# ppjian19/PhoreGen

Measured on AMD Instinct MI355X. Metric: denoise-steps/sec (batch=128, ~40-atom graphs), higher is better.
Workload: dtype f32; 1 GPU; BASELINE.json configs[2]: ONE batch of 128 LigPhore-shaped graphs (n~N(40,6) atoms, p~N(107,30) pharmacophore nodes), partitioned over 1 GPU(s) by the fitted step cost, steps t=999.. of the 1000-step sampler, device Philox noise, trajectory written; graphs_total=128, graphs_rank0=128, n_ctx=18401, n_lig=5115, e_knn=588832, e_bond=203720, e3=8087028, parallelism=graph-sharded x1, final RCCL gather only, triplet_workgroups_rank0=256

## Files before the change

### include/phoregen_hip.h

```cpp
#ifndef PHOREGEN_HIP_H
#define PHOREGEN_HIP_H

#include <stdint.h>

#ifdef __cplusplus
extern "C" {
#endif

const char* pg_last_error(void);
int pg_abi_version(void);
int pg_abi_struct_sizes(int* out, int n);

int pg_order_point_create(void** ev);
int pg_order_point_destroy(void* ev);
int pg_order_point_record(void* ev, void* stream);
int pg_order_point_wait(void* ev, void* stream);
int pg_debug_order_point_fence_free(int on);

enum {
  PG_OP_RECORD = 0, PG_OP_WAIT = 1, PG_OP_GEMM = 2, PG_OP_SEG_ATTN = 3, PG_OP_EMBED_CTX = 4, PG_OP_EMBED_BOND = 5, PG_OP_KNN_CTX = 6,
  PG_OP_LIG_NORMALS = 7, PG_OP_EDGE_GATE = 8, PG_OP_KNN_GROUP_BY_KIND = 9, PG_OP_BOND_SMEAR = 10, PG_OP_ATTN_FOLD_QUERY = 11,
  PG_OP_ATTN_UNFOLD_VALUE = 12, PG_OP_APPLY_DX = 13, PG_OP_LAYER_GEOM = 14, PG_OP_ROWS_LINEAR = 15, PG_OP_ATOM_COUNT = 16,
  PG_OP_EMBED_BOND_E16 = 17
};
// ... 12 lines not shown
int pg_program_destroy(void* prog);

int pg_micro_mfma_f32(int workgroups, int iters, float* sink, double* flops, void* stream);

int pg_selftest_mfma(int* d_result, void* stream);
int pg_selftest_philox(const uint32_t* ctr_key, int n, uint32_t* out, void* stream);
int pg_debug_force_generic_seg(int mask);

typedef struct {
  const float* X;   int ldx;  int K1;
  const float* X2;  int ldx2; int K2;
  const float* W;   int ldw;
  const float* bias;
  const float* ln_gamma; const float* ln_beta;
  const float* add1; int ld_add1; const int* idx1;
  const float* add2; int ld_add2; const int* idx2;
  float out_scale;
  int   act;
  float* Y; int ldy; int M; int N;
  const int* rows;
  int add_rows;
  int row_extent;
  const int* tile_rows;
} PgGemm;
int pg_gemm(const PgGemm* p, void* stream);
int pg_debug_gemm_streaming(int on);
int pg_gemm_is_streaming(const PgGemm* p);

typedef struct {
  int n_graphs, n_ctx, n_lig, n_phore, n_bond;
  int max_nlig;
  int max_gctx;
  const int* g_ctx_off;
  const int* g_nph;
  const int* g_nlig;
  const int* g_eid_off;
  const int* eid;
  const int* ctx_graph;
  const uint8_t* ctx_is_lig;
  const int* lig2ctx;
  const int* bond_src;
  const int* bond_dst;
  const int* bond_desc;
  const int* g_bond_off;
  const int* edge_ref;
} PgTopo;
// ... 492 lines not shown
```

### phoregen_amd/csrc/gemm.hip

```cpp
#include <stdlib.h>

#include "common.h"
#include "../../include/phoregen_hip.h"

namespace pg {

constexpr int BM = 128, BN = 128, BK = 32, LDT = BK + 1;


__global__ __launch_bounds__(256) void gemm_kernel(PgGemm p PG_ABL_PARAM) {
  __shared__ __attribute__((aligned(16))) float smem[(BM + BN) * LDT];
  float* const As = smem;
  float* const Bs = smem + BM * LDT;
  __shared__ float rstat[BM * 2];

  const int tid = threadIdx.x, lane = tid & 63, wave = tid >> 6;
  const int col0 = blockIdx.x * BN;
  const int K = p.K1 + p.K2;
  for (int rb = blockIdx.y; rb * BM < p.M; rb += gridDim.y) {
  const int row0 = rb * BM;
  const int wr = (wave >> 1) * 64, wc = (wave & 1) * 64;
  const bool ln = p.ln_gamma != nullptr;

  if (ln) {
// ... 197 lines not shown
      const int src = rows ? rows[grow] : grow;
      *reinterpret_cast<f4*>(xs + r * RL_LD + 4 * c4) = __builtin_nontemporal_load(reinterpret_cast<const f4*>(X + (size_t)src * ldx) + c4);
    }
    __syncthreads();
    f4 acc = {bias, bias, bias, bias};
    const float* xa = xs + (16 * wave + m) * RL_LD + g;
#pragma unroll
    for (int s_ = 0; s_ < 32; ++s_) acc = mfma16(xa[4 * s_], wr[s_], acc);
    if (m < n_out) {
#pragma unroll
      for (int r = 0; r < 4; ++r) {
        const int grow = row0 + 16 * wave + 4 * g + r;
        if (grow < M) Y[(size_t)grow * ldy + m] = acc[r];
      }
    }
  }
}

}

namespace pg {
bool gemm_stream_eligible(const PgGemm* p);
bool gemm_stream_windows_ok(const PgGemm* p);
int launch_gemm_stream(const PgGemm* p, hipStream_t st);
}

static int g_gemm_stream = 1;
extern "C" int pg_debug_gemm_streaming(int on) { const int old = g_gemm_stream; g_gemm_stream = on; return old; }

extern "C" int pg_gemm_is_streaming(const PgGemm* p) {
  return p && (p->tile_rows || (g_gemm_stream && pg::gemm_stream_eligible(p))) ? 1 : 0;
}

extern "C" int pg_gemm(const PgGemm* p, void* stream) {
  if (!p || !p->X || !p->W || !p->Y || p->M < 0 || p->N <= 0) { pg::set_error("pg_gemm: bad arguments"); return PG_ERR_ARG; }
  if (p->M == 0) return PG_OK;
  if (p->K2 > 0 && !p->X2) { pg::set_error("pg_gemm: K2 > 0 without X2"); return PG_ERR_ARG; }
  if (p->ln_gamma && !p->ln_beta) { pg::set_error("pg_gemm: ln_gamma without ln_beta"); return PG_ERR_ARG; }
  if (p->ln_gamma && (p->K2 != 0 || p->K1 != 128 || (p->ldx & 3) || ((size_t)p->X & 15))) { pg::set_error("pg_gemm: LayerNorm-on-load needs K1 == 128, K2 == 0, 16-byte aligned rows"); return PG_ERR_ARG; }
  if (p->tile_rows) {
    if (!pg::gemm_stream_windows_ok(p)) {
      pg::set_error("pg_gemm: tile_rows needs the streaming kernel's plain or LayerNorm-on-load form (K1 = 128, K2 = 0, no added operand, "
                    "no rows, act = 0, N a multiple of 128), M = 64 x windows and row_extent >= 64 (M %d, N %d, K1 %d, K2 %d, row_extent %d)",
                    p->M, p->N, p->K1, p->K2, p->row_extent);
      return PG_ERR_ARG;
    }
    hipPointerAttribute_t at;
    if (hipPointerGetAttributes(&at, p->tile_rows) != hipSuccess || at.type == hipMemoryTypeUnregistered) {
      (void)hipGetLastError();
      pg::set_error("pg_gemm: tile_rows is not device-accessible memory");
      return PG_ERR_ARG;
    }
    if (at.type == hipMemoryTypeHost || at.type == hipMemoryTypeManaged) {
      const int* o = p->tile_rows;
      for (int t = 0; t < p->M / 64; ++t)
        if (o[t] < 0 || o[t] > p->row_extent - 64) {
          pg::set_error("pg_gemm: tile_rows[%d] = %d outside [0, row_extent - 64 = %d]", t, o[t], p->row_extent - 64);
          return PG_ERR_ARG;
        }
    }
    return pg::launch_gemm_stream(p, (hipStream_t)stream);
  }
// ... 22 lines not shown
```

### phoregen_amd/csrc/gemm_stream.hip

```cpp
#include <type_traits>

#include "wave_prims.h"
#include "../../include/phoregen_hip.h"

namespace pg {

typedef int i2v __attribute__((ext_vector_type(2)));

constexpr int ST_BM = 64;
constexpr int ST_STAGE = ST_BM * 128 * 4;

template <int NW , int NADD , int K1 ,
          int K2 , bool LN ,
          bool SSP = false ,
          bool WIN = false >
__global__ __launch_bounds__(NW * 64, NW == 4 ? 2 : 1) void gemm_stream_kernel(PgGemm p, int n_tiles) {
  extern __shared__ __attribute__((aligned(1024))) char st_lds[];
  const int lane = threadIdx.x & 63;
  const int wave = __builtin_amdgcn_readfirstlane(threadIdx.x >> 6);
  const int l31 = lane & 31, kh = lane >> 5;
  const int colw = blockIdx.y * (NW * 32) + 32 * wave;
  const int col = colw + l31;

  constexpr bool DMA = K1 == 128;
  static_assert((K1 == 128 || K1 == 16 || K1 == 0) && (K2 == 20 || K2 == 0) && K1 + K2 > 0, "K1 128 | 16 | 0, K2 20 | 0");
  float Wr[DMA ? 64 : 1];
  if constexpr (DMA) {
    const float* wrow = p.W + (size_t)col * p.ldw + 4 * kh;
#pragma unroll
    for (int c = 0; c < 16; ++c) {
      const f4 w = *reinterpret_cast<const f4*>(wrow + 8 * c);
#pragma unroll
      for (int e = 0; e < 4; ++e) Wr[4 * c + e] = w[e];
    }
  }
  float W2r[K2 ? 10 : 1];
  if constexpr (K2 > 0) {
#pragma unroll
    for (int s2 = 0; s2 < 10; ++s2) W2r[s2] = p.W[(size_t)col * p.ldw + K1 + 10 * kh + s2];
  }
  const unsigned ldx2b = (unsigned)p.ldx2 * 4u;
  const __amdgpu_buffer_rsrc_t descX2 = __builtin_amdgcn_make_buffer_rsrc(const_cast<float*>(K2 ? p.X2 : nullptr), 0, (unsigned)p.M * ldx2b, 0x00020000);
  const unsigned voffX2 = (unsigned)l31 * ldx2b + 40u * kh;
  float xa[2][10], xb[2][10];
  auto load_x2 = [&](unsigned row0, float (&x)[2][10]) {
#pragma unroll
    for (int b = 0; b < 2; ++b) {
      const unsigned so = (row0 + 32u * b) * ldx2b;
      const i4v v0 = __builtin_amdgcn_raw_buffer_load_b128(descX2, voffX2, so, 0);
      const i4v v1 = __builtin_amdgcn_raw_buffer_load_b128(descX2, voffX2 + 16u, so, 0);
      const i2v v2 = __builtin_amdgcn_raw_buffer_load_b64(descX2, voffX2 + 32u, so, 0);
#pragma unroll
      for (int e = 0; e < 4; ++e) { x[b][e] = __builtin_bit_cast(float, (int)v0[e]); x[b][4 + e] = __builtin_bit_cast(float, (int)v1[e]); }
      x[b][8] = __builtin_bit_cast(float, (int)v2[0]);
      x[b][9] = __builtin_bit_cast(float, (int)v2[1]);
    }
// ... 1 lines not shown
  float W1r[K1 == 16 ? 8 : 1];
  float xra[2][8], xrb[2][8];
  const unsigned ldxrb = K1 == 16 ? (unsigned)p.ldx * 4u : 0u;
  const __amdgpu_buffer_rsrc_t descXr = __builtin_amdgcn_make_buffer_rsrc(const_cast<float*>(K1 == 16 ? p.X : nullptr), 0, (unsigned)p.M * ldxrb, 0x00020000);
  const unsigned voffXr = (unsigned)l31 * ldxrb + 32u * kh;
  if constexpr (K1 == 16) {
#pragma unroll
    for (int s1 = 0; s1 < 8; ++s1) W1r[s1] = p.W[(size_t)col * p.ldw + 8 * kh + s1];
  }
  auto load_xr = [&](unsigned row0, float (&x)[2][8]) {
#pragma unroll
    for (int b = 0; b < 2; ++b) {
      const unsigned so = (row0 + 32u * b) * ldxrb;
      const i4v v0 = __builtin_amdgcn_raw_buffer_load_b128(descXr, voffXr, so, 0);
      const i4v v1 = __builtin_amdgcn_raw_buffer_load_b128(descXr, voffXr + 16u, so, 0);
#pragma unroll
      for (int e = 0; e < 4; ++e) { x[b][e] = __builtin_bit_cast(float, (int)v0[e]); x[b][4 + e] = __builtin_bit_cast(float, (int)v1[e]); }
    }
  };
  const float bias = p.bias ? p.bias[col] : 0.f;
  f16v biasv;
#pragma unroll
  for (int r = 0; r < 16; ++r) biasv[r] = bias;

  const f4* const lnt = reinterpret_cast<const f4*>(st_lds + 2 * ST_STAGE);
  if constexpr (LN) {
    float* t = reinterpret_cast<float*>(st_lds + 2 * ST_STAGE);
    if (threadIdx.x < 128) { t[threadIdx.x] = p.ln_gamma[threadIdx.x]; t[128 + threadIdx.x] = p.ln_beta[threadIdx.x]; }
    __syncthreads();
  }

  const unsigned ldxb = (unsigned)p.ldx * 4u, ldyb = (unsigned)p.ldy * 4u;
  const unsigned n_rows = WIN ? (unsigned)p.row_extent : (unsigned)p.M;
  const i4v descX = raw_buffer_desc(p.X, n_rows * ldxb);
  const __amdgpu_buffer_rsrc_t descY = __builtin_amdgcn_make_buffer_rsrc(p.Y, 0, n_rows * ldyb, 0x00020000);
  const unsigned row_sub = lane >> 3, pp = lane & 7;
  const unsigned voff_even = row_sub * ldxb + ((pp ^ ((row_sub >> 1) & 7u)) << 4);
  const unsigned voff_odd = row_sub * ldxb + ((pp ^ ((4u + (row_sub >> 1)) & 7u)) << 4);
  const unsigned voff_wave = (wave & 1) ? voff_odd : voff_even;
  unsigned rd[4];
#pragma unroll
  for (int q = 0; q < 4; ++q)
    rd[q] = (unsigned)(l31 >> 3) * 4096u + (unsigned)(l31 & 7) * 128u + (((unsigned)(2 * q + kh) ^ ((unsigned)(l31 >> 1) & 7u)) << 4);
  unsigned voffY[4];
#pragma unroll
  for (int t = 0; t < 4; ++t) voffY[t] = (unsigned)(4 * kh + t) * ldyb + (unsigned)l31 * 4u;

  f16v g1[2];
  const __amdgpu_buffer_rsrc_t descI1 = __builtin_amdgcn_make_buffer_rsrc(const_cast<int*>(NADD ? p.idx1 : nullptr), 0, (unsigned)p.M * 4u, 0x00020000);
// ... 49 lines not shown
        lds_dma_1k(stage * ST_STAGE + ((unsigned)wave * 4u + j) * 1024u, voff_wave, descX, row0b + (unsigned)wave * 8u * ldxb + j * 128u);
    }
  };

  if constexpr (K1 == 16) load_xr(tile_row0(tile), xra);
  if constexpr (K2 > 0) load_x2(tile_row0(tile), xa);
  unsigned wrow = 0, wrow_next = 0;
  if constexpr (WIN) { wrow = win_row0(tile); wrow_next = win_row0(tile + tile_step); }
  if constexpr (DMA) dma_tile(WIN ? wrow : tile_row0(tile), 0);
  if constexpr (NADD == 1) { i4v ix[8]; load_idx(descI1, tile_row0(tile), ix); gather(descA1, ld1b, ix, g1); }
  if constexpr (NADD == 2) gather_plain(tile_row0(tile), g1);

  auto body = [&](auto stage_c, auto first_c) {
    constexpr unsigned stage = decltype(stage_c)::value;
    constexpr bool first = decltype(first_c)::value;
    if constexpr (DMA) {
      if constexpr (first) asm volatile("s_waitcnt vmcnt(0)\n\ts_barrier" ::: "memory");
      else asm volatile("s_waitcnt vmcnt(32)\n\ts_barrier" ::: "memory");
    }
    const unsigned next = tile + tile_step;
    float (&xc)[2][10] = stage ? xb : xa;
    float (&xn)[2][10] = stage ? xa : xb;
    i4v ix1[8];
    if constexpr (NADD == 1) load_idx(descI1, tile_row0(next), ix1);
    if constexpr (K1 == 16) load_xr(tile_row0(next), stage ? xra : xrb);
    if constexpr (K2 > 0) load_x2(tile_row0(next), xn);
    unsigned wrow_after = 0;
    if constexpr (WIN) wrow_after = win_row0(next + tile_step);
    if constexpr (DMA) dma_tile(WIN ? wrow_next : tile_row0(next), stage ^ 1u);

    if constexpr (LN) {
      const unsigned row = threadIdx.x >> 2, jj = threadIdx.x & 3;
      char* const base = st_lds + stage * ST_STAGE + ((row >> 3) * 4u + jj) * 1024u + (row & 7u) * 128u;
      const unsigned sw = (row >> 1) & 7u;
      f4 v[8];
#pragma unroll
      for (int q = 0; q < 8; ++q) v[q] = *reinterpret_cast<const f4*>(base + 16 * (q ^ sw));
      float sm = 0.f;
#pragma unroll
      for (int q = 0; q < 8; ++q) sm += (v[q][0] + v[q][1]) + (v[q][2] + v[q][3]);
      sm += __shfl_xor(sm, 1);
      sm += __shfl_xor(sm, 2);
      const float mu = sm * (1.f / 128.f);
      float qs = 0.f;
#pragma unroll
      for (int q = 0; q < 8; ++q)
#pragma unroll
// ... 19 lines not shown
      for (int b = 0; b < 2; ++b)
#pragma unroll
        for (int r = 0; r < 16; ++r) acc[b][r] = g1[b][r] + bias;
    } else {
      acc[0] = biasv;
      acc[1] = biasv;
    }

    if constexpr (K1 == 16) {
      float (&xrc)[2][8] = stage ? xrb : xra;
#pragma unroll
      for (int s1 = 0; s1 < 8; ++s1) {
        acc[0] = mfma32(xrc[0][s1], W1r[s1], acc[0]);
        acc[1] = mfma32(xrc[1][s1], W1r[s1], acc[1]);
      }
    }
    if constexpr (K2 > 0) {
#pragma unroll
      for (int s2 = 0; s2 < 10; ++s2) {
        acc[0] = mfma32(xc[0][s2], W2r[s2], acc[0]);
        acc[1] = mfma32(xc[1][s2], W2r[s2], acc[1]);
      }
    }
    if constexpr (DMA) {
      auto frag = [&](int c, int b) {
        return *reinterpret_cast<const f4*>(st_lds + rd[c & 3] + (stage * ST_STAGE + b * 16384u + (c >> 2) * 1024u));
      };
      f4 aA0 = frag(0, 0), aA1 = frag(0, 1), aB0, aB1;
#pragma unroll
      for (int c = 0; c < 16; c += 2) {
        if (c == 12) {
          if constexpr (NADD == 1) gather(descA1, ld1b, ix1, g1);
          if constexpr (NADD == 2) gather_plain(tile_row0(next), g1);
        }
        aB0 = frag(c + 1, 0); aB1 = frag(c + 1, 1);
        __builtin_amdgcn_sched_barrier(0);
#pragma unroll
        for (int e = 0; e < 4; ++e) {
          acc[0] = mfma32(aA0[e], Wr[4 * c + e], acc[0]);
          acc[1] = mfma32(aA1[e], Wr[4 * c + e], acc[1]);
        }
        if (c + 2 < 16) { aA0 = frag(c + 2, 0); aA1 = frag(c + 2, 1); }
        __builtin_amdgcn_sched_barrier(0);
#pragma unroll
        for (int e = 0; e < 4; ++e) {
          acc[0] = mfma32(aB0[e], Wr[4 * c + 4 + e], acc[0]);
          acc[1] = mfma32(aB1[e], Wr[4 * c + 4 + e], acc[1]);
        }
      }
      __builtin_amdgcn_sched_barrier(0);
    } else {
      if constexpr (NADD == 1) gather(descA1, ld1b, ix1, g1);
      if constexpr (NADD == 2) gather_plain(tile_row0(next), g1);
    }

    const unsigned row0 = WIN ? wrow : tile_row0(tile);
#pragma unroll
    for (int b = 0; b < 2; ++b)
#pragma unroll
      for (int r = 0; r < 16; ++r) {
        const unsigned soff = (row0 + 32u * b + 8u * (r >> 2)) * ldyb + (unsigned)colw * 4u;
        float v = acc[b][r];
        if constexpr (LN) v *= p.out_scale;
        if constexpr (SSP) v = ssp(v);
        __builtin_amdgcn_raw_buffer_store_b32(__builtin_bit_cast(int, v), descY, voffY[r & 3], soff, 0);
      }
    tile = next;
    if constexpr (WIN) { wrow = wrow_next; wrow_next = wrow_after; }
  };

  body(std::integral_constant<unsigned, 0>{}, std::true_type{});
  while ((int)tile < n_tiles) {
    body(std::integral_constant<unsigned, 1>{}, std::false_type{});
    if ((int)tile >= n_tiles) break;
    body(std::integral_constant<unsigned, 0>{}, std::false_type{});
  }
  asm volatile("s_waitcnt vmcnt(0)" ::: "memory");
}

template <int NW, int NADD, int K1, int K2, bool LN = false, bool SSP = false, bool WIN = false>
static int launch_stream_t(const PgGemm* p, hipStream_t st) {
  const void* k = reinterpret_cast<const void*>(gemm_stream_kernel<NW, NADD, K1, K2, LN, SSP, WIN>);
  const size_t lds = K1 == 128 ? 2 * ST_STAGE + (LN ? 1024 : 0) : 0;
  if (lds) if (int rc = reserve_lds(k, lds, "pg_gemm(stream)")) return rc;
  const int n_tiles = (p->M + ST_BM - 1) / ST_BM;
  const int n_cb = p->N / (NW * 32);
  int per_cb = (NW == 4 ? 2 : 1) * kNumCU / n_cb;
  if (per_cb < 1) per_cb = 1;
  if (per_cb > n_tiles) per_cb = n_tiles;
  hipLaunchKernelGGL((gemm_stream_kernel<NW, NADD, K1, K2, LN, SSP, WIN>), dim3(per_cb, n_cb), dim3(NW * 64), lds, st, *p, n_tiles);
  return check_launch("pg_gemm(stream)");
}

bool gemm_stream_eligible(const PgGemm* p) {
  const bool k128 = p->K1 == 128 && (p->K2 == 0 || p->K2 == 20), k20 = p->K1 == 20 && p->K2 == 0, k16 = p->K1 == 16 && (p->K2 == 0 || p->K2 == 20);
  if (!(k128 || k20 || k16) || p->rows || (p->N & 127) || p->M < ST_BM) return false;
  if (p->act == 1) { if (p->K1 != 128 || p->K2 || p->N != 128 || p->ln_gamma || p->add1 || p->add2 || p->out_scale != 1.0f) return false; }
  else if (p->act != 0) return false;
  if (p->ln_gamma) { if (p->K1 != 128 || p->K2 || p->N != 128 || p->add1 || p->add2) return false; }
  else if (p->out_scale != 1.0f) return false;
  if ((p->ldx & 3) || ((size_t)p->X & 15) || (p->ldw & 3) || ((size_t)p->W & 15)) return false;
  if (p->K2 && ((p->ldx2 & 1) || ((size_t)p->X2 & 7))) return false;
  if (k20 && (p->ldx & 1)) return false;
  if (p->add2) return false;
  if (p->add1 && p->idx1 && (p->add_rows <= 0 || (size_t)p->add_rows * p->ld_add1 * 4 >= 0xfffff000ull)) return false;
  if (p->add1 && !p->idx1 && ((size_t)p->M * p->ld_add1 * 4 >= 0xfffff000ull || p->add1 == p->Y)) return false;
  if ((size_t)p->M * p->ldx * 4 >= 0xfffff000ull || (size_t)p->M * p->ldy * 4 >= 0xfffff000ull) return false;
  return true;
}

template <int K1, int K2>
static int launch_stream_k(const PgGemm* p, hipStream_t st) {
  const bool wide = (p->N & 255) == 0;
  const int nadd = p->add1 ? (p->idx1 ? 1 : 2) : 0;
  if (wide) {
    if (nadd == 0) return launch_stream_t<8, 0, K1, K2>(p, st);
    if (nadd == 1) return launch_stream_t<8, 1, K1, K2>(p, st);
    return launch_stream_t<8, 2, K1, K2>(p, st);
  }
  if (nadd == 0) return launch_stream_t<4, 0, K1, K2>(p, st);
  if (nadd == 1) return launch_stream_t<4, 1, K1, K2>(p, st);
  return launch_stream_t<4, 2, K1, K2>(p, st);
}

bool gemm_stream_windows_ok(const PgGemm* p) {
  if (p->K1 != 128 || p->K2 || p->add1 || p->add2 || p->rows || p->act != 0 || (p->N & 127)) return false;
  if (p->M < ST_BM || (p->M % ST_BM) || p->row_extent < ST_BM) return false;
  if ((size_t)p->row_extent * p->ldx * 4 >= 0xfffff000ull || (size_t)p->row_extent * p->ldy * 4 >= 0xfffff000ull) return false;
  return gemm_stream_eligible(p);
}

int launch_gemm_stream(const PgGemm* p, hipStream_t st) {
  if (p->tile_rows) {
    if (p->ln_gamma) return launch_stream_t<4, 0, 128, 0, true, false, true>(p, st);
    return (p->N & 255) == 0 ? launch_stream_t<8, 0, 128, 0, false, false, true>(p, st) : launch_stream_t<4, 0, 128, 0, false, false, true>(p, st);
  }
  if (p->ln_gamma) return launch_stream_t<4, 0, 128, 0, true>(p, st);
  if (p->act == 1) return launch_stream_t<4, 0, 128, 0, false, true>(p, st);
  if (p->K1 == 20) {
    PgGemm q = *p;
    q.X2 = p->X; q.ldx2 = p->ldx; q.K2 = 20; q.K1 = 0;
    return launch_stream_k<0, 20>(&q, st);
  }
  if (p->K1 == 16) return p->K2 ? launch_stream_k<16, 20>(p, st) : launch_stream_k<16, 0>(p, st);
  return p->K2 ? launch_stream_k<128, 20>(p, st) : launch_stream_k<128, 0>(p, st);
}

}
```

### phoregen_amd/engine.py

```python
import ctypes as C

import torch

from . import hip, options
from .packing import HEAD_SCALE, ModelPack


_SIDE_STREAMS = {}


_TRI_GRID_CACHE = {}


def side_streams(device_index, stream_set=0):
    key = (device_index, stream_set)
    if key not in _SIDE_STREAMS:
        with torch.cuda.device(device_index):
            _SIDE_STREAMS[key] = [torch.cuda.Stream(), torch.cuda.Stream(), torch.cuda.Stream()]
    return _SIDE_STREAMS[key]


def _f(*shape, device, zero=False):
    return (torch.zeros if zero else torch.empty)(*shape, dtype=torch.float32, device=device)

# ... 16 lines not shown
        self.dev = plan.device
        self._keep = []
        self.debug = None
        self.timers = None
        self.trace = None
        self.tri_calls = []
        o = options.snapshot()
        self.multi_stream = o['streams']
        self.layer_ahead = o['layer_ahead']
        self.tri_split, self.tri_split_from = o['tri_split'], o['tri_split_from']
        self.tri_overlap = o['tri_overlap']
        self.chain_q_from = o['chain_q_from']
        self.tune_grid = o['tune_grid']
        self.tuned_tri_grid = None
        self.geom_split = o['geom_split'] == 'always' or (o['geom_split'] == 'auto' and self.plan.n_bond < o['geom_split_below'])
        self.ahead_v2 = o['ahead_v2'] == 'always' or (o['ahead_v2'] == 'auto' and self.plan.n_bond < o['ahead_v2_below'])
        self.step_ahead = o['step_ahead']
        self.pos_tiled, self.pos_tiled_below = o['pos_tiled'], o['pos_tiled_below']
        self.tri_grid = o['tri_grid']
        self.lig_windows = o['lig_windows'] if plan.lig_windows is not None else 0
        self.l0_compact = bool(o['l0_compact']) and full and not phore_only
        if self.l0_compact and not hasattr(pack.layers[0].TB, 'W_hbg36'):
            raise ValueError('phoregen_amd: l0_compact needs the composed layer-0 weights of the sampler pack (ModelPack(..., detach=True))')
        self._lane = 0
        self._n_points = 0
        self._points = {}
        self.c_program = o['c_program']
        self._compiled = {}
        self._side = None
        self.stream_set = 0
        self._alloc()
        if full:
            self.prog_phore = self._build_phore_program()
            if not phore_only:
                self.prog_fwd = self._build_forward_program()
                self.prog_step = self.prog_ahead = None

    def _alloc(self):
        p, d = self.plan, self.dev
        n, E, k = p.n_ctx, p.n_bond, self.k
        w = self.ws = type('WS', (), {})()
        w.in_h_node, w.in_pos = _f(p.n_lig, 12, device=d), _f(p.n_lig, 3, device=d)
        w.in_h_edge = _f(E, 6, device=d)
        w.in_t = torch.zeros(p.n_graphs, dtype=torch.int64, device=d)
        w.in_t_next = torch.zeros(p.n_graphs, dtype=torch.int64, device=d)
        w.h_phore_ctx, w.x_phore_ctx = _f(n, 18, device=d, zero=True), _f(n, 3, device=d, zero=True)
# ... 82 lines not shown
        if tap.kind == 'order':
            for what, pt, lane in tap.ops:
                ev = self._points.get(pt)
                if ev is None:
                    ev = self._points[pt] = hip.OrderPoint()
                if what == 'record':
                    ev.record(streams[lane])
                else:
                    ev.wait(streams[lane])
        elif tap.kind == 'event':
            if self.timers is not None:
                ev = torch.cuda.Event(enable_timing=True)
                ev.record(streams[tap.lane])
                self.timers.setdefault(tap.name, []).append((tap.start, ev))
        elif self.debug is not None:
            with torch.cuda.stream(streams[tap.lane]):
                self.debug[tap.name] = tuple(t.clone() for t in tap.tensors)

    def kernel_ms(self, name):
        evs = self.timers.get(name, [])
        return [a.elapsed_time(b) for (sa, a), (sb, b) in zip(evs[0::2], evs[1::2]) if sa and not sb]

    def _gemm(self, prog, X, K1, W, Y, M, N, bias=None, X2=None, K2=0, ln=None, add1=None, idx1=None, add2=None,
              idx2=None, scale=1.0, act=hip.ACT_NONE, rows=None, lig_only=False):
        g = hip.PgGemm()
        g.X, g.ldx, g.K1 = X.data_ptr(), X.stride(0), K1
        g.X2, g.ldx2, g.K2 = (X2.data_ptr(), X2.stride(0), K2) if X2 is not None else (None, 0, 0)
        g.W, g.ldw = W.data_ptr(), W.stride(0)
        g.bias = hip.ptr(bias)
        g.ln_gamma, g.ln_beta = (ln[0].data_ptr(), ln[1].data_ptr()) if ln is not None else (None, None)
        g.add1, g.ld_add1, g.idx1 = (add1.data_ptr(), add1.stride(0), hip.ptr(idx1)) if add1 is not None else (None, 0, None)
        g.add2, g.ld_add2, g.idx2 = (add2.data_ptr(), add2.stride(0), hip.ptr(idx2)) if add2 is not None else (None, 0, None)
        g.out_scale, g.act = scale, act
        g.Y, g.ldy, g.M, g.N = Y.data_ptr(), Y.stride(0), M, N
        g.rows = hip.ptr(rows)
        g.add_rows = add1.size(0) if add1 is not None else 0
        if lig_only and self.lig_windows:
            g.tile_rows, g.row_extent, g.M = self.plan.lig_windows.data_ptr(), M, 64 * self.plan.n_lig_windows
        self._keep += [g, X, W, Y, bias, X2, ln, add1, idx1, add2, idx2, rows]
        self._call(prog, self.lib.pg_gemm, C.byref(g))

    def _seg(self, prog, mode, n_seg, seg_ids, a, **kw):
        s = hip.PgSegAttn()
        s.mode, s.n_seg, s.seg_ids = mode, n_seg, hip.ptr(seg_ids)
        s.knn_k = self.k
        s.ln_gk, s.ln_bk, s.ln_gv, s.ln_bv = (t.data_ptr() for t in (a.ln_gk, a.ln_bk, a.ln_gv, a.ln_bv))
        for key, val in kw.items():
            setattr(s, key, val.data_ptr() if torch.is_tensor(val) else val)
            self._keep.append(val)
        self._keep += [s, seg_ids, a]
        s.form_name = hip.form_name(hip.seg_form(self.plan.topo_ref, s))
        self._call(prog, self.lib.pg_seg_attn, self.plan.topo_ref, C.byref(s))

    def _query_gemm(self, prog, a, Y, col0, h_dst_lists, buf):
        n, wq = self.plan.n_ctx, self.ws.q[buf]
        qh = Y[:, col0 + 4 * 128: col0 + 5 * 128]
        lig_only = all(is_lig for _, _, is_lig in h_dst_lists)
        self._gemm(prog, qh, 128, a.W2q, wq, n, 128, bias=a.b2q, ln=(a.q_ln_g, a.q_ln_b), scale=HEAD_SCALE, lig_only=lig_only)

    def _node_attention(self, prog, mode, a, Y, col0, x, h_dst_lists, out=None, dx=None, csrc=None, buf=0, extra=None,
                        query_done=False, qbuf=None):
        w, p, n = self.ws, self.plan, self.plan.n_ctx
# ... 105 lines not shown
        def node_head(h_final):
            W0, b0, W2, b2 = pk.v0
            self._gemm(prog, h_final, 128, W0, w.head, n, 128, bias=b0, act=hip.ACT_SSP)
            self._call(prog, lib.pg_rows_linear, w.head.data_ptr(), 128, 128, W2.data_ptr(), b2.data_ptr(), 12, p.n_lig,
                       p.lig2ctx.data_ptr(), w.out_v.data_ptr(), 12)
        self._denoiser_program(prog, lig, both, heads=(bond_head, node_head), pre_join=None if step_ahead else (2,), step_ahead=step_ahead)
        return prog

    def _build_ahead_program(self):
        w, p, pk, prog = self.ws, self.plan, self.pack, []
        lig = [(p.lig2ctx, p.n_lig, True)]
        both = [(p.lig2ctx, p.n_lig, True), (p.phore2ctx, p.n_phore, False)]
        L0 = pk.layers[0]
        self._sync(prog, 3, (2,))
        self._lane = 3
        self._embed_bond(prog, w.in_t_next)
        hb_done = self._record(prog, 3)
        self._lane = 2
        self._embed_ctx(prog, w.in_t_next, coords=False)
        self._first_layer_gemm(prog, L0, w.h_in, w.Y1)
        y1_done = self._record(prog, 2)
        self._query_gemm(prog, L0.NE, w.Y1, 0, both, 3)
        self._wait(prog, 2, hb_done)
        self._triplet_queries(prog, L0, w.hb[0], w.Y1, l0=True)
        self._lane = 3
        self._wait(prog, 3, y1_done)
        self._bond_node_rows(prog, L0, w.hb[0], w.Y1, l0=True)
        self._node_attention(prog, hip.SEG_BOND_NODE, L0.NB, w.Y1, 5 * 128, w.x[0], lig, out=w.aggB, csrc=w.CsB2, buf=2)
        self._lane = 0
        return prog

    def pipelined_programs(self):
        if not (self.step_ahead and self.multi_stream and self.layer_ahead and self.plan.n_tri_iters):
            return None
        if self.prog_step is None:
            tri_calls, self.tri_calls = self.tri_calls, []
            self.prog_step = self._build_forward_program(step_ahead=True)
            self.step_tri_calls, self.tri_calls = self.tri_calls, tri_calls
            self.prog_ahead = self._build_ahead_program()
        return self.prog_step, self.prog_ahead

    def _first_layer_gemm(self, prog, L, h_in, Y1):
        p, n = self.plan, self.plan.n_ctx
        if not self.lig_windows:
            self._gemm(prog, h_in, 128, L.W_node1, Y1, n, 1920, bias=L.b_node1)
            return
        self._gemm(prog, h_in, 128, L.W_node1[:640], Y1[:, :640], n, 640, bias=L.b_node1[:640])
        self._gemm(prog, h_in, 128, L.W_node1[640:], Y1[:, 640:], n, 1280, bias=L.b_node1[640:], lig_only=True)

    def _l0_rows(self, l0, hb_in, W, W16):
        return (self.ws.e16, 16, W16) if (l0 and self.l0_compact) else (hb_in, 128, W)

    def _triplet_rows(self, prog, L, hb_in, Y1, staged, l0=False):
        w, p, E = self.ws, self.plan, self.plan.n_bond
        X, K, W = self._l0_rows(l0, hb_in, L.TB.W_hbg, L.TB.W_hbg36 if l0 and self.l0_compact else None)
        self._gemm(prog, X, K, W, w.P, E, 256, X2=w.G, K2=20, add1=Y1[:, 10 * 128:12 * 128], idx1=p.bond_src,
                   **({} if staged else dict(add2=Y1[:, 12 * 128:14 * 128], idx2=p.bond_dst)))

    def _triplet_queries(self, prog, L, hb_in, Y1, l0=False):
        w, p, E = self.ws, self.plan, self.plan.n_bond
        X, K, W = self._l0_rows(l0, hb_in, L.TB.W_q_hb, L.TB.W_q_hb16 if l0 and self.l0_compact else None)
        self._gemm(prog, X, K, W, w.qhid, E, 128, add1=Y1[:, 14 * 128:15 * 128], idx1=p.bond_dst)
        self._gemm(prog, w.qhid, 128, L.TB.W2q, w.qT, E, 128, bias=L.TB.b2q, ln=(L.TB.q_ln_g, L.TB.q_ln_b), scale=HEAD_SCALE)

    def _bond_node_rows(self, prog, L, hb_in, Y1, l0=False):
        w, p, E = self.ws, self.plan, self.plan.n_bond
        X, K, W = self._l0_rows(l0, hb_in, L.NB.W_hb, L.NB.W_hb16 if l0 and self.l0_compact else None)
        self._gemm(prog, X, K, W, w.CsB2, E, 256, add1=Y1[:, 7 * 128:9 * 128], idx1=p.bond_src)

    def _denoiser_program(self, prog, lig, both, heads=None, pre_join=None, step_ahead=False):
        w, p, pk, lib = self.ws, self.plan, self.pack, self.lib
        n, E, t = p.n_ctx, p.n_bond, p.topo_ref
        h, x, hb = w.h, w.x, w.hb
        g = pk.gate
        self._fork(prog, (1,))
        self._lane = 1
        self._call(prog, lib.pg_knn_ctx, t, x[0].data_ptr(), self.k, w.nbr.data_ptr(), w.deg.data_ptr())
        self._call(prog, lib.pg_edge_gate, t, x[0].data_ptr(), w.nbr.data_ptr(), w.deg.data_ptr(), self.k,
                   g['W0'].data_ptr(), g['b0'].data_ptr(), g['g'].data_ptr(), g['b'].data_ptr(), g['W3'].data_ptr(),
                   C.c_float(g['b3']), w.ew.data_ptr())
        self._mark(prog, 'graph', w.nbr, w.deg, w.ew, lane=1)
        self._call(prog, lib.pg_knn_group_by_kind, t, self.k, w.nbr.data_ptr(), w.deg.data_ptr(), w.ew.data_ptr())
        self._lane = 0
        cur = 0
        staged = bool(p.n_tri_iters)
        n_layers = len(pk.layers)
        ahead = self.layer_ahead and self.multi_stream
        v2 = self.ahead_v2 and ahead
        chain_q = self.multi_stream and (v2 or E >= self.chain_q_from)
        tri_grid = self.tri_grid if self.tri_grid >= 0 else ((192 if E < 15000 else 224 if E < 80000 else 0) if self.multi_stream else 0)
        self._tune = None
        if (self.tune_grid and self.tri_grid < 0 and self.multi_stream and staged and 0 < tri_grid <= 224):
            self._tune = dict(cands=[g for g in (tri_grid, tri_grid + 32, tri_grid - 32) if 128 <= g <= 256])

        if v2 and w.Y1b is None:
            w.Y1b = torch.empty_like(w.Y1)
        split = v2 and self.geom_split
        if split and getattr(w, 'x_node', None) is None:
            w.x_node = [torch.empty_like(x[0]), torch.empty_like(x[0])]
            w.dxe2 = torch.zeros_like(w.dxe)

        first_layer_gemm = lambda L_, h_in, Y1_: self._first_layer_gemm(prog, L_, h_in, Y1_)
        triplet_queries = lambda L_, hb_in, Y1_, l0=False: self._triplet_queries(prog, L_, hb_in, Y1_, l0)
        bond_node_rows = lambda L_, hb_in, Y1_, l0=False: self._bond_node_rows(prog, L_, hb_in, Y1_, l0)
        assert not step_ahead or (ahead and staged)

        for li, L in enumerate(pk.layers):
            nxt = 1 - cur
            hc, xc, hbc, hn, xn, hbn = (w.h_in if li == 0 else h[cur]), x[cur], hb[cur], h[nxt], x[nxt], hb[nxt]
            Y1c, Y1n = (w.Y1, w.Y1) if not v2 else ((w.Y1, w.Y1b) if li % 2 == 0 else (w.Y1b, w.Y1))
            xc1 = w.x_node[cur] if (split and li > 0) else xc
            dxe = w.dxe2 if (split and li % 2) else w.dxe
            pre = ahead and (li > 0 or step_ahead)
            pre0 = step_ahead and li == 0
            if li == 0:
                self._call(prog, lib.pg_layer_geom, t, xc.data_ptr(), None, None, w.nrm_phore_ctx.data_ptr(), None,
                           w.nrm.data_ptr(), w.G.data_ptr())
            late2 = self.lig_windows == 2 and pre and not v2 and not pre0
            if late2:
                self._wait(prog, 0, y1_done)
            elif (pre and not v2) or pre0:
                self._sync(prog, 0, (2,))
            elif not pre:
                first_layer_gemm(L, hc, Y1c)
            if li == 0 and pre_join:
                self._join(prog, pre_join)
# ... 409 lines not shown
```

### phoregen_amd/hip.py

```python
import ctypes as C
import struct
import sys
import os

import torch

_HERE = os.path.dirname(os.path.abspath(__file__))
LIB_PATH = os.path.join(_HERE, '_lib', 'libphoregen_hip.so')

c_fp = C.c_void_p
c_ip = C.c_void_p


class PgGemm(C.Structure):
    _fields_ = [('X', c_fp), ('ldx', C.c_int), ('K1', C.c_int),
                ('X2', c_fp), ('ldx2', C.c_int), ('K2', C.c_int),
                ('W', c_fp), ('ldw', C.c_int),
                ('bias', c_fp),
                ('ln_gamma', c_fp), ('ln_beta', c_fp),
                ('add1', c_fp), ('ld_add1', C.c_int), ('idx1', c_ip),
                ('add2', c_fp), ('ld_add2', C.c_int), ('idx2', c_ip),
                ('out_scale', C.c_float), ('act', C.c_int),
                ('Y', c_fp), ('ldy', C.c_int), ('M', C.c_int), ('N', C.c_int), ('rows', c_ip), ('add_rows', C.c_int),
                ('row_extent', C.c_int), ('tile_rows', c_ip)]


class PgTopo(C.Structure):
    _fields_ = [('n_graphs', C.c_int), ('n_ctx', C.c_int), ('n_lig', C.c_int), ('n_phore', C.c_int),
                ('n_bond', C.c_int), ('max_nlig', C.c_int), ('max_gctx', C.c_int),
                ('g_ctx_off', c_ip), ('g_nph', c_ip), ('g_nlig', c_ip), ('g_eid_off', c_ip), ('eid', c_ip),
                ('ctx_graph', c_ip), ('ctx_is_lig', c_ip), ('lig2ctx', c_ip), ('bond_src', c_ip),
                ('bond_dst', c_ip), ('bond_desc', c_ip), ('g_bond_off', c_ip), ('edge_ref', c_ip)]


class PgSegAttn(C.Structure):
    _fields_ = [('mode', C.c_int), ('n_seg', C.c_int), ('seg_ids', c_ip), ('seg_chunks', c_ip),
                ('x', c_fp), ('nrm', c_fp), ('nbr', c_ip), ('deg', c_ip), ('ew', c_fp), ('knn_k', C.c_int),
                ('Csrc_k', c_fp), ('Csrc_v', c_fp), ('ld_csrc', C.c_int),
                ('Cdst_k', c_fp), ('Cdst_v', c_fp), ('ld_cdst', C.c_int),
                ('Wf_k', c_fp), ('Wf_v', c_fp), ('Wg2_k', c_fp), ('Wg2_v', c_fp), ('G', c_fp),
                ('ln_gk', c_fp), ('ln_bk', c_fp), ('ln_gv', c_fp), ('ln_bv', c_fp),
                ('U', c_fp), ('q', c_fp), ('W2k_l', c_fp), ('W2v_l', c_fp), ('b2v', c_fp),
                ('W2xv_l', c_fp), ('b2xv', c_fp),
                ('S', c_fp), ('swn', c_fp), ('resid', c_fp), ('out', c_fp), ('dx', c_fp),
                ('accumulate_dx', C.c_int), ('alpha', c_fp), ('alpha_rows', C.c_int), ('efeat', c_fp), ('efeat_off', c_ip),
                ('tri_iters', c_ip), ('n_tri_iters', C.c_int), ('tri_counter', c_ip),
                ('seg_ids2', c_ip), ('n_seg2', C.c_int), ('Wf_k2', c_fp), ('Wf_v2', c_fp), ('tri_grid', C.c_int), ('pos_tiled', C.c_int), ('tri_max_nlig', C.c_int)]
# ... 339 lines not shown
```

### phoregen_amd/options.py

```python
import contextlib
import os

DEFAULTS = dict(
    streams=True,
    layer_ahead=True,
    ahead_v2='auto',
    ahead_v2_below=82000,
    pos_tiled='auto',
    pos_tiled_below=1500,
    step_ahead=True,
    c_program=True,
    geom_split='auto',
    geom_split_below=16000,
    tune_grid=True,
    chain_q_from=150000,
    tri_split=True,
    tri_split_from=82000,
    tri_overlap=3,
    lig_windows=2,
    tri_grid=-1,
    l0_compact=True,
    dgrad_mm=True,
    rows_sum=True,
    tri_onepass=True,
    wide_gemm=True,
    bwd_atom_sort=True,
    bwd_split='all',
    bwd_grid=256,
    tri_bwd_form=2,
    tri_bwd_grid=256,
    ph_onepass=True,
)

_tri = lambda v: {'0': 'never', '1': 'auto', '2': 'always'}[v]
_flag = lambda v: v != '0'
_ENV = {
    'PG_STREAMS': ('streams', _flag),
    'PG_LAYER_AHEAD': ('layer_ahead', _flag), 'PG_AHEAD_V2': ('ahead_v2', _tri), 'PG_AHEAD_V2_BELOW': ('ahead_v2_below', int), 'PG_TRI_GRID': ('tri_grid', int), 'PG_POS_TILED': ('pos_tiled', _tri), 'PG_POS_TILED_BELOW': ('pos_tiled_below', int), 'PG_C_PROGRAM': ('c_program', _flag), 'PG_STEP_AHEAD': ('step_ahead', _flag), 'PG_CHAIN_Q_FROM': ('chain_q_from', int), 'PG_TRI_SPLIT': ('tri_split', _flag), 'PG_TUNE_GRID': ('tune_grid', _flag), 'PG_GEOM_SPLIT': ('geom_split', _tri), 'PG_LIG_WINDOWS': ('lig_windows', int), 'PG_L0_COMPACT': ('l0_compact', _flag),
    'PG_DGRAD_MM': ('dgrad_mm', _flag),
    'PG_ROWS_SUM': ('rows_sum', _flag), 'PG_TRI_ONEPASS': ('tri_onepass', _flag), 'PG_WIDE_GEMM': ('wide_gemm', _flag), 'PG_BWD_GRID': ('bwd_grid', int), 'PG_BWD_SPLIT': ('bwd_split', lambda v: {'0': 'none', '1': 'knn', '2': 'all'}[v]), 'PG_BWD_ATOM_SORT': ('bwd_atom_sort', _flag),
    'PG_TRI_BWD_FORM': ('tri_bwd_form', int), 'PG_TRI_BWD_GRID': ('tri_bwd_grid', int), 'PG_PH_ONEPASS': ('ph_onepass', _flag),
}
_overrides = {}


def get(name):
    if name in _overrides:
        return _overrides[name]
    if os.environ.get('PHOREGEN_DEBUG') == '1':
        for var, (key, conv) in _ENV.items():
            if key == name and var in os.environ:
                return conv(os.environ[var])
    return DEFAULTS[name]


def snapshot():
    return {k: get(k) for k in DEFAULTS}


@contextlib.contextmanager
def override(**kw):
# ... 11 lines not shown
```

Before: 57.89 steps/s.

## Fuse triplet query two-layer MLP into one streaming GEMM kernel

Adds a two-layer (chained) form to the streaming GEMM. The first product plus gathered add goes to LDS, then LayerNorm+ReLU runs in LDS and the second 128x128 product is applied in the same kernel. The triplet-query path now uses it instead of writing the hidden activation qhid to global memory and reading it back in a second GEMM launch. This trades one launch and the E x 128 round trip for more registers (a second 64-float weight fragment), which may lower occupancy. The next tile's gather is also moved so it overlaps the second product.

```diff
diff --git a/include/phoregen_hip.h b/include/phoregen_hip.h
--- a/include/phoregen_hip.h
+++ b/include/phoregen_hip.h
@@ -58,6 +58,7 @@
   int add_rows;
   int row_extent;
   const int* tile_rows;
+  const float* W2; int ldw2; const float* bias2;
 } PgGemm;
 int pg_gemm(const PgGemm* p, void* stream);
 int pg_debug_gemm_streaming(int on);
diff --git a/phoregen_amd/csrc/gemm.hip b/phoregen_amd/csrc/gemm.hip
--- a/phoregen_amd/csrc/gemm.hip
+++ b/phoregen_amd/csrc/gemm.hip
@@ -243,6 +243,7 @@
 namespace pg {
 bool gemm_stream_eligible(const PgGemm* p);
 bool gemm_stream_windows_ok(const PgGemm* p);
+bool gemm_stream_chain_ok(const PgGemm* p);
 int launch_gemm_stream(const PgGemm* p, hipStream_t st);
 }
 
@@ -250,7 +251,7 @@
 extern "C" int pg_debug_gemm_streaming(int on) { const int old = g_gemm_stream; g_gemm_stream = on; return old; }
 
 extern "C" int pg_gemm_is_streaming(const PgGemm* p) {
-  return p && (p->tile_rows || (g_gemm_stream && pg::gemm_stream_eligible(p))) ? 1 : 0;
+  return p && (p->tile_rows || p->W2 || (g_gemm_stream && pg::gemm_stream_eligible(p))) ? 1 : 0;
 }
 
 extern "C" int pg_gemm(const PgGemm* p, void* stream) {
@@ -258,7 +259,15 @@
   if (p->M == 0) return PG_OK;
   if (p->K2 > 0 && !p->X2) { pg::set_error("pg_gemm: K2 > 0 without X2"); return PG_ERR_ARG; }
   if (p->ln_gamma && !p->ln_beta) { pg::set_error("pg_gemm: ln_gamma without ln_beta"); return PG_ERR_ARG; }
-  if (p->ln_gamma && (p->K2 != 0 || p->K1 != 128 || (p->ldx & 3) || ((size_t)p->X & 15))) { pg::set_error("pg_gemm: LayerNorm-on-load needs K1 == 128, K2 == 0, 16-byte aligned rows"); return PG_ERR_ARG; }
+  if (p->ln_gamma && !p->W2 && (p->K2 != 0 || p->K1 != 128 || (p->ldx & 3) || ((size_t)p->X & 15))) { pg::set_error("pg_gemm: LayerNorm-on-load needs K1 == 128, K2 == 0, 16-byte aligned rows"); return PG_ERR_ARG; }
+  if (p->W2) {
+    if (!pg::gemm_stream_chain_ok(p)) {
+      pg::set_error("pg_gemm: the two-layer form (W2) needs N = 128, K1 = 128 or 16, K2 = 0, at least 64 rows, ln_gamma / ln_beta, add1 only with "
+                    "idx1, no rows / tile_rows / add2 / act, 16-byte aligned rows (M %d, N %d, K1 %d, K2 %d, act %d)", p->M, p->N, p->K1, p->K2, p->act);
+      return PG_ERR_ARG;
+    }
+    return pg::launch_gemm_stream(p, (hipStream_t)stream);
+  }
   if (p->tile_rows) {
     if (!pg::gemm_stream_windows_ok(p)) {
       pg::set_error("pg_gemm: tile_rows needs the streaming kernel's plain or LayerNorm-on-load form (K1 = 128, K2 = 0, no added operand, "
diff --git a/phoregen_amd/csrc/gemm_stream.hip b/phoregen_amd/csrc/gemm_stream.hip
--- a/phoregen_amd/csrc/gemm_stream.hip
+++ b/phoregen_amd/csrc/gemm_stream.hip
@@ -9,11 +9,72 @@
 
 constexpr int ST_BM = 64;
 constexpr int ST_STAGE = ST_BM * 128 * 4;
+
+template <class Hook>
+__device__ __forceinline__ void st_product(const char* stage, const unsigned (&rd)[4], const float (&Wp)[64], f16v (&acc)[2], Hook hook) {
+  auto frag = [&](int c, int b) { return *reinterpret_cast<const f4*>(stage + rd[c & 3] + (b * 16384u + (c >> 2) * 1024u)); };
+  f4 aA0 = frag(0, 0), aA1 = frag(0, 1), aB0, aB1;
+#pragma unroll
+  for (int c = 0; c < 16; c += 2) {
+    hook(c);
+    aB0 = frag(c + 1, 0); aB1 = frag(c + 1, 1);
+    __builtin_amdgcn_sched_barrier(0);
+#pragma unroll
+    for (int e = 0; e < 4; ++e) {
+      acc[0] = mfma32(aA0[e], Wp[4 * c + e], acc[0]);
+      acc[1] = mfma32(aA1[e], Wp[4 * c + e], acc[1]);
+    }
+    if (c + 2 < 16) { aA0 = frag(c + 2, 0); aA1 = frag(c + 2, 1); }
+    __builtin_amdgcn_sched_barrier(0);
+#pragma unroll
+    for (int e = 0; e < 4; ++e) {
+      acc[0] = mfma32(aB0[e], Wp[4 * c + 4 + e], acc[0]);
+      acc[1] = mfma32(aB1[e], Wp[4 * c + 4 + e], acc[1]);
+    }
+  }
+  __builtin_amdgcn_sched_barrier(0);
+}
+
+__device__ __forceinline__ void st_ln_relu_tile(char* stage, const f4* lnt) {
+  unsigned tid = threadIdx.x;
+  asm volatile("" : "+v"(tid));
+  const unsigned row = tid >> 2, jj = tid & 3;
+  char* const base = stage + ((row >> 3) * 4u + jj) * 1024u + (row & 7u) * 128u;
+  const unsigned sw = (row >> 1) & 7u;
+  f4 v[8];
+#pragma unroll
+  for (int q = 0; q < 8; ++q) v[q] = *reinterpret_cast<const f4*>(base + 16 * (q ^ sw));
+  float sm = 0.f;
+#pragma unroll
+  for (int q = 0; q < 8; ++q) sm += (v[q][0] + v[q][1]) + (v[q][2] + v[q][3]);
+  sm += __shfl_xor(sm, 1);
+  sm += __shfl_xor(sm, 2);
+  const float mu = sm * (1.f / 128.f);
+  float qs = 0.f;
+#pragma unroll
+  for (int q = 0; q < 8; ++q)
+#pragma unroll
+    for (int e = 0; e < 4; ++e) { const float d = v[q][e] - mu; qs = fmaf(d, d, qs); }
+  qs += __shfl_xor(qs, 1);
+  qs += __shfl_xor(qs, 2);
+  const float rs = 1.0f / sqrtf(qs * (1.f / 128.f) + 1e-5f);
+#pragma unroll
+  for (int q = 0; q < 8; ++q) {
+    const unsigned k4 = 8u * jj + (unsigned)q;
+    const f4 ga = lnt[k4], be = lnt[32 + k4];
+    f4 o;
+#pragma unroll
+    for (int e = 0; e < 4; ++e) o[e] = fmaxf((v[q][e] - mu) * rs * ga[e] + be[e], 0.f);
+    *reinterpret_cast<f4*>(base + 16 * (q ^ sw)) = o;
+  }
+  asm volatile("s_waitcnt lgkmcnt(0)\n\ts_barrier" ::: "memory");
+}
 
 template <int NW , int NADD , int K1 ,
           int K2 , bool LN ,
           bool SSP = false ,
-          bool WIN = false >
+          bool WIN = false ,
+          bool CH = false >
 __global__ __launch_bounds__(NW * 64, NW == 4 ? 2 : 1) void gemm_stream_kernel(PgGemm p, int n_tiles) {
   extern __shared__ __attribute__((aligned(1024))) char st_lds[];
   const int lane = threadIdx.x & 63;
@@ -24,6 +85,7 @@
 
   constexpr bool DMA = K1 == 128;
   static_assert((K1 == 128 || K1 == 16 || K1 == 0) && (K2 == 20 || K2 == 0) && K1 + K2 > 0, "K1 128 | 16 | 0, K2 20 | 0");
+  static_assert(!CH || (NW == 4 && NADD <= 1 && (K1 == 128 || K1 == 16) && K2 == 0 && !LN && !SSP && !WIN), "two-layer form: 4 waves, K1 128 | 16");
   float Wr[DMA ? 64 : 1];
   if constexpr (DMA) {
     const float* wrow = p.W + (size_t)col * p.ldw + 4 * kh;
@@ -32,6 +94,16 @@
       const f4 w = *reinterpret_cast<const f4*>(wrow + 8 * c);
 #pragma unroll
       for (int e = 0; e < 4; ++e) Wr[4 * c + e] = w[e];
+    }
+  }
+  float Wc[CH ? 64 : 1];
+  if constexpr (CH) {
+    const float* wrow = p.W2 + (size_t)col * p.ldw2 + 4 * kh;
+#pragma unroll
+    for (int c = 0; c < 16; ++c) {
+      const f4 w = *reinterpret_cast<const f4*>(wrow + 8 * c);
+#pragma unroll
+      for (int e = 0; e < 4; ++e) Wc[4 * c + e] = w[e];
     }
   }
   float W2r[K2 ? 10 : 1];
@@ -79,9 +151,10 @@
   f16v biasv;
 #pragma unroll
   for (int r = 0; r < 16; ++r) biasv[r] = bias;
+  const float bias2 = CH && p.bias2 ? p.bias2[col] : 0.f;
 
   const f4* const lnt = reinterpret_cast<const f4*>(st_lds + 2 * ST_STAGE);
-  if constexpr (LN) {
+  if constexpr (LN || CH) {
     float* t = reinterpret_cast<float*>(st_lds + 2 * ST_STAGE);
     if (threadIdx.x < 128) { t[threadIdx.x] = p.ln_gamma[threadIdx.x]; t[128 + threadIdx.x] = p.ln_beta[threadIdx.x]; }
     __syncthreads();
@@ -177,7 +250,7 @@
     float (&xc)[2][10] = stage ? xb : xa;
     float (&xn)[2][10] = stage ? xa : xb;
     i4v ix1[8];
-    if constexpr (NADD == 1) load_idx(descI1, tile_row0(next), ix1);
+    if constexpr (NADD == 1 && !CH) load_idx(descI1, tile_row0(next), ix1);
     if constexpr (K1 == 16) load_xr(tile_row0(next), stage ? xra : xrb);
     if constexpr (K2 > 0) load_x2(tile_row0(next), xn);
     unsigned wrow_after = 0;
@@ -243,7 +316,9 @@
         acc[1] = mfma32(xc[1][s2], W2r[s2], acc[1]);
       }
     }
-    if constexpr (DMA) {
+    if constexpr (CH && DMA) {
+      st_product(st_lds + stage * ST_STAGE, rd, Wr, acc, [](int) {});
+    } else if constexpr (DMA) {
       auto frag = [&](int c, int b) {
         return *reinterpret_cast<const f4*>(st_lds + rd[c & 3] + (stage * ST_STAGE + b * 16384u + (c >> 2) * 1024u));
       };
@@ -270,9 +345,53 @@
         }
       }
       __builtin_amdgcn_sched_barrier(0);
-    } else {
+    } else if constexpr (!CH) {
       if constexpr (NADD == 1) gather(descA1, ld1b, ix1, g1);
       if constexpr (NADD == 2) gather_plain(tile_row0(next), g1);
+    }
+
+    if constexpr (CH) {
+      if constexpr (DMA) asm volatile("s_barrier" ::: "memory");
+      unsigned hl = (unsigned)lane;
+      asm volatile("" : "+v"(hl));
+      const unsigned hkh = hl >> 5;
+      char* const hbase = st_lds + stage * ST_STAGE + (unsigned)wave * 1024u + hkh * 512u + (hl & 3u) * 4u;
+      const unsigned hslot = ((hl & 31u) >> 2) ^ (2u * hkh);
+#pragma unroll
+      for (int b = 0; b < 2; ++b)
+#pragma unroll
+        for (int r = 0; r < 16; ++r) {
+          const unsigned sw = 4u * ((r >> 2) & 1) + ((r & 3) >> 1);
+          const float v = acc[b][r];
+          *reinterpret_cast<float*>(hbase + (4 * b + (r >> 2)) * 4096u + (r & 3) * 128u + ((hslot ^ sw) << 4)) = v;
+        }
+      asm volatile("s_waitcnt lgkmcnt(0)\n\ts_barrier" ::: "memory");
+      auto load_idx_half = [&](int b) {
+#pragma unroll
+        for (int e = 4 * b; e < 4 * b + 4; ++e) ix1[e] = __builtin_amdgcn_raw_buffer_load_b128(descI1, 16u * kh, (tile_row0(next) + 8u * e) * 4u, 0);
+      };
+      st_ln_relu_tile(st_lds + stage * ST_STAGE, lnt);
+      float b2 = bias2;
+      asm volatile("" : "+v"(b2));
+#pragma unroll
+      for (int b = 0; b < 2; ++b)
+#pragma unroll
+        for (int r = 0; r < 16; ++r) acc[b][r] = b2;
+      st_product(st_lds + stage * ST_STAGE, rd, Wc, acc, [&](int c) {
+        if constexpr (NADD == 1) {
+          if (c == 0) load_idx_half(0);
+          if (c == 6 || c == 12) {
+            const int b = c == 12;
+#pragma unroll
+            for (int q = 0; q < 4; ++q)
+#pragma unroll
+              for (int t = 0; t < 4; ++t)
+                g1[b][4 * q + t] = __builtin_bit_cast(
+                    float, __builtin_amdgcn_raw_buffer_load_b32(descA1, (unsigned)ix1[4 * b + q][t] * ld1b + colb, 0, 0));
+          }
+          if (c == 6) load_idx_half(1);
+        }
+      });
     }
 
     const unsigned row0 = WIN ? wrow : tile_row0(tile);
@@ -282,7 +401,7 @@
       for (int r = 0; r < 16; ++r) {
         const unsigned soff = (row0 + 32u * b + 8u * (r >> 2)) * ldyb + (unsigned)colw * 4u;
         float v = acc[b][r];
-        if constexpr (LN) v *= p.out_scale;
+        if constexpr (LN || CH) v *= p.out_scale;
         if constexpr (SSP) v = ssp(v);
         __builtin_amdgcn_raw_buffer_store_b32(__builtin_bit_cast(int, v), descY, voffY[r & 3], soff, 0);
       }
@@ -299,17 +418,17 @@
   asm volatile("s_waitcnt vmcnt(0)" ::: "memory");
 }
 
-template <int NW, int NADD, int K1, int K2, bool LN = false, bool SSP = false, bool WIN = false>
+template <int NW, int NADD, int K1, int K2, bool LN = false, bool SSP = false, bool WIN = false, bool CH = false>
 static int launch_stream_t(const PgGemm* p, hipStream_t st) {
-  const void* k = reinterpret_cast<const void*>(gemm_stream_kernel<NW, NADD, K1, K2, LN, SSP, WIN>);
-  const size_t lds = K1 == 128 ? 2 * ST_STAGE + (LN ? 1024 : 0) : 0;
+  const void* k = reinterpret_cast<const void*>(gemm_stream_kernel<NW, NADD, K1, K2, LN, SSP, WIN, CH>);
+  const size_t lds = (K1 == 128 || CH) ? 2 * ST_STAGE + ((LN || CH) ? 1024 : 0) : 0;
   if (lds) if (int rc = reserve_lds(k, lds, "pg_gemm(stream)")) return rc;
   const int n_tiles = (p->M + ST_BM - 1) / ST_BM;
   const int n_cb = p->N / (NW * 32);
   int per_cb = (NW == 4 ? 2 : 1) * kNumCU / n_cb;
   if (per_cb < 1) per_cb = 1;
   if (per_cb > n_tiles) per_cb = n_tiles;
-  hipLaunchKernelGGL((gemm_stream_kernel<NW, NADD, K1, K2, LN, SSP, WIN>), dim3(per_cb, n_cb), dim3(NW * 64), lds, st, *p, n_tiles);
+  hipLaunchKernelGGL((gemm_stream_kernel<NW, NADD, K1, K2, LN, SSP, WIN, CH>), dim3(per_cb, n_cb), dim3(NW * 64), lds, st, *p, n_tiles);
   return check_launch("pg_gemm(stream)");
 }
 
@@ -351,7 +470,20 @@
   return gemm_stream_eligible(p);
 }
 
+bool gemm_stream_chain_ok(const PgGemm* p) {
+  if (!p->W2 || p->N != 128 || p->K2 || p->X2 || p->rows || p->tile_rows || p->add2 || p->act != 0 || p->M < ST_BM) return false;
+  if (p->K1 != 128 && p->K1 != 16) return false;
+  if (!p->ln_gamma || !p->ln_beta || (p->add1 && !p->idx1)) return false;
+  PgGemm q = *p;
+  q.W2 = nullptr; q.ln_gamma = q.ln_beta = nullptr; q.out_scale = 1.0f;
+  return gemm_stream_eligible(&q) && !(p->ldw2 & 3) && !((size_t)p->W2 & 15);
+}
+
 int launch_gemm_stream(const PgGemm* p, hipStream_t st) {
+  if (p->W2) {
+    if (p->K1 == 16) return p->add1 ? launch_stream_t<4, 1, 16, 0, false, false, false, true>(p, st) : launch_stream_t<4, 0, 16, 0, false, false, false, true>(p, st);
+    return p->add1 ? launch_stream_t<4, 1, 128, 0, false, false, false, true>(p, st) : launch_stream_t<4, 0, 128, 0, false, false, false, true>(p, st);
+  }
   if (p->tile_rows) {
     if (p->ln_gamma) return launch_stream_t<4, 0, 128, 0, true, false, true>(p, st);
     return (p->N & 255) == 0 ? launch_stream_t<8, 0, 128, 0, false, false, true>(p, st) : launch_stream_t<4, 0, 128, 0, false, false, true>(p, st);
diff --git a/phoregen_amd/engine.py b/phoregen_amd/engine.py
--- a/phoregen_amd/engine.py
+++ b/phoregen_amd/engine.py
@@ -62,6 +62,7 @@
         self.l0_compact = bool(o['l0_compact']) and full and not phore_only
         if self.l0_compact and not hasattr(pack.layers[0].TB, 'W_hbg36'):
             raise ValueError('phoregen_amd: l0_compact needs the composed layer-0 weights of the sampler pack (ModelPack(..., detach=True))')
+        self.gemm_chain = bool(o['gemm_chain']) and full and not phore_only
         self._lane = 0
         self._n_points = 0
         self._points = {}
@@ -190,7 +191,7 @@
         return [a.elapsed_time(b) for (sa, a), (sb, b) in zip(evs[0::2], evs[1::2]) if sa and not sb]
 
     def _gemm(self, prog, X, K1, W, Y, M, N, bias=None, X2=None, K2=0, ln=None, add1=None, idx1=None, add2=None,
-              idx2=None, scale=1.0, act=hip.ACT_NONE, rows=None, lig_only=False):
+              idx2=None, scale=1.0, act=hip.ACT_NONE, rows=None, lig_only=False, then=None):
         g = hip.PgGemm()
         g.X, g.ldx, g.K1 = X.data_ptr(), X.stride(0), K1
         g.X2, g.ldx2, g.K2 = (X2.data_ptr(), X2.stride(0), K2) if X2 is not None else (None, 0, 0)
@@ -205,7 +206,9 @@
         g.add_rows = add1.size(0) if add1 is not None else 0
         if lig_only and self.lig_windows:
             g.tile_rows, g.row_extent, g.M = self.plan.lig_windows.data_ptr(), M, 64 * self.plan.n_lig_windows
-        self._keep += [g, X, W, Y, bias, X2, ln, add1, idx1, add2, idx2, rows]
+        if then is not None:
+            g.W2, g.ldw2, g.bias2 = then[0].data_ptr(), then[0].stride(0), hip.ptr(then[1])
+        self._keep += [g, X, W, Y, bias, X2, ln, add1, idx1, add2, idx2, rows, then]
         self._call(prog, self.lib.pg_gemm, C.byref(g))
 
     def _seg(self, prog, mode, n_seg, seg_ids, a, **kw):
@@ -357,7 +360,7 @@
         y1_done = self._record(prog, 2)
         self._query_gemm(prog, L0.NE, w.Y1, 0, both, 3)
         self._wait(prog, 2, hb_done)
-        self._triplet_queries(prog, L0, w.hb[0], w.Y1, l0=True)
+        self._triplet_queries(prog, L0, w.hb[0], w.Y1, l0=True, chain=self.gemm_chain)
         self._lane = 3
         self._wait(prog, 3, y1_done)
         self._bond_node_rows(prog, L0, w.hb[0], w.Y1, l0=True)
@@ -392,9 +395,13 @@
         self._gemm(prog, X, K, W, w.P, E, 256, X2=w.G, K2=20, add1=Y1[:, 10 * 128:12 * 128], idx1=p.bond_src,
                    **({} if staged else dict(add2=Y1[:, 12 * 128:14 * 128], idx2=p.bond_dst)))
 
-    def _triplet_queries(self, prog, L, hb_in, Y1, l0=False):
+    def _triplet_queries(self, prog, L, hb_in, Y1, l0=False, chain=False):
         w, p, E = self.ws, self.plan, self.plan.n_bond
         X, K, W = self._l0_rows(l0, hb_in, L.TB.W_q_hb, L.TB.W_q_hb16 if l0 and self.l0_compact else None)
+        if chain and E >= 64:
+            self._gemm(prog, X, K, W, w.qT, E, 128, add1=Y1[:, 14 * 128:15 * 128], idx1=p.bond_dst, ln=(L.TB.q_ln_g, L.TB.q_ln_b),
+                       then=(L.TB.W2q, L.TB.b2q), scale=HEAD_SCALE)
+            return
         self._gemm(prog, X, K, W, w.qhid, E, 128, add1=Y1[:, 14 * 128:15 * 128], idx1=p.bond_dst)
         self._gemm(prog, w.qhid, 128, L.TB.W2q, w.qT, E, 128, bias=L.TB.b2q, ln=(L.TB.q_ln_g, L.TB.q_ln_b), scale=HEAD_SCALE)
 
@@ -436,7 +443,7 @@
             w.dxe2 = torch.zeros_like(w.dxe)
 
         first_layer_gemm = lambda L_, h_in, Y1_: self._first_layer_gemm(prog, L_, h_in, Y1_)
-        triplet_queries = lambda L_, hb_in, Y1_, l0=False: self._triplet_queries(prog, L_, hb_in, Y1_, l0)
+        triplet_queries = lambda L_, hb_in, Y1_, l0=False: self._triplet_queries(prog, L_, hb_in, Y1_, l0, chain=self.gemm_chain)
         bond_node_rows = lambda L_, hb_in, Y1_, l0=False: self._bond_node_rows(prog, L_, hb_in, Y1_, l0)
         assert not step_ahead or (ahead and staged)
 
diff --git a/phoregen_amd/hip.py b/phoregen_amd/hip.py
--- a/phoregen_amd/hip.py
+++ b/phoregen_amd/hip.py
@@ -22,7 +22,8 @@
                 ('add2', c_fp), ('ld_add2', C.c_int), ('idx2', c_ip),
                 ('out_scale', C.c_float), ('act', C.c_int),
                 ('Y', c_fp), ('ldy', C.c_int), ('M', C.c_int), ('N', C.c_int), ('rows', c_ip), ('add_rows', C.c_int),
-                ('row_extent', C.c_int), ('tile_rows', c_ip)]
+                ('row_extent', C.c_int), ('tile_rows', c_ip),
+                ('W2', c_fp), ('ldw2', C.c_int), ('bias2', c_fp)]
 
 
 class PgTopo(C.Structure):
diff --git a/phoregen_amd/options.py b/phoregen_amd/options.py
--- a/phoregen_amd/options.py
+++ b/phoregen_amd/options.py
@@ -20,6 +20,7 @@
     lig_windows=2,
     tri_grid=-1,
     l0_compact=True,
+    gemm_chain=True,
     dgrad_mm=True,
     rows_sum=True,
     tri_onepass=True,
@@ -37,6 +38,7 @@
 _ENV = {
     'PG_STREAMS': ('streams', _flag),
     'PG_LAYER_AHEAD': ('layer_ahead', _flag), 'PG_AHEAD_V2': ('ahead_v2', _tri), 'PG_AHEAD_V2_BELOW': ('ahead_v2_below', int), 'PG_TRI_GRID': ('tri_grid', int), 'PG_POS_TILED': ('pos_tiled', _tri), 'PG_POS_TILED_BELOW': ('pos_tiled_below', int), 'PG_C_PROGRAM': ('c_program', _flag), 'PG_STEP_AHEAD': ('step_ahead', _flag), 'PG_CHAIN_Q_FROM': ('chain_q_from', int), 'PG_TRI_SPLIT': ('tri_split', _flag), 'PG_TUNE_GRID': ('tune_grid', _flag), 'PG_GEOM_SPLIT': ('geom_split', _tri), 'PG_LIG_WINDOWS': ('lig_windows', int), 'PG_L0_COMPACT': ('l0_compact', _flag),
+    'PG_GEMM_CHAIN': ('gemm_chain', _flag),
     'PG_DGRAD_MM': ('dgrad_mm', _flag),
     'PG_ROWS_SUM': ('rows_sum', _flag), 'PG_TRI_ONEPASS': ('tri_onepass', _flag), 'PG_WIDE_GEMM': ('wide_gemm', _flag), 'PG_BWD_GRID': ('bwd_grid', int), 'PG_BWD_SPLIT': ('bwd_split', lambda v: {'0': 'none', '1': 'knn', '2': 'all'}[v]), 'PG_BWD_ATOM_SORT': ('bwd_atom_sort', _flag),
     'PG_TRI_BWD_FORM': ('tri_bwd_form', int), 'PG_TRI_BWD_GRID': ('tri_bwd_grid', int), 'PG_PH_ONEPASS': ('ph_onepass', _flag),
```

Result: no change. 58.47 steps/s (median of 6 runs) (+1.0%).
